# technosaurus/PDMP3

Hardware: AMD Instinct MI355X
Metric: MP3 frames/sec (44.1 kHz stereo 320 kbps), transforms-only hot path (higher is better)
Workload: dtype f32; 1 GPU; C2 (BASELINE configs[1]): 2048 stereo frames = 4096 granules per GPU per step, pre-Huffman-decoded spectra resident in HBM, one stream; frames_per_gpu=2048, granules_per_gpu=4096, seed=0x5eed0000c2, chunk_frames=auto

## Files before the change

pdmp3_amd/csrc/decode_core.h:

```cpp
#pragma once

#include <math.h>
#include <stdint.h>
#include <string.h>
#include "../../include/pdmp3_hip.h"

namespace pdmp3 {
struct ConstBank;
}

#if defined(__HIPCC__)
#define PD_FN __device__ __forceinline__
#define PD_SLOW_FN __device__ __attribute__((noinline))
#define PD_MFN __device__ __forceinline__
#define PD_HD __host__ __device__ __forceinline__
#define PD_FMA(a, b, c) __builtin_fmaf((a), (b), (c))
#define PD_CLOCK() __builtin_amdgcn_s_memtime()
#define PD_UNROLL _Pragma("unroll")
#define PD_UNROLL_N(n) _Pragma(PD_STR_(unroll n))
#define PD_STR_(x) #x
#define PD_NOUNROLL _Pragma("nounroll")
#define PD_SCHED_FENCE() __builtin_amdgcn_sched_barrier(0)
#define PD_PIN(x) asm volatile("" : "+v"(x))
#define PD_ANY(c) (__builtin_amdgcn_ballot_w64(c) != 0ull)
#define PD_LANE() ((int)(threadIdx.x & 63))
#define PD_UNIFORM(x) __builtin_amdgcn_readfirstlane((int)(x))
#define PD_SHFL_XOR(v, m) __shfl_xor((v), (m))
#define PD_WAVE_SYNC()                                       \
  __builtin_amdgcn_fence(__ATOMIC_RELEASE, "wavefront");    \
  __builtin_amdgcn_wave_barrier();                          \
  __builtin_amdgcn_fence(__ATOMIC_ACQUIRE, "wavefront")
#define PD_STORE_DEVICE(p, v) __hip_atomic_store((p), (v), __ATOMIC_RELAXED, __HIP_MEMORY_SCOPE_AGENT)
#define PD_LOAD_DEVICE(p) __hip_atomic_load((p), __ATOMIC_RELAXED, __HIP_MEMORY_SCOPE_AGENT)
#define PD_VMEM_DRAIN() asm volatile("s_waitcnt vmcnt(0)" ::: "memory")
#define PD_SLEEP() __builtin_amdgcn_s_sleep(4)
#define PD_SETPRIO(x) __builtin_amdgcn_s_setprio(x)
#define PD_LDS_FLAG(p) (*(volatile __attribute__((address_space(3))) unsigned*)(p))
#define PD_BALLOT(c) ((unsigned long long)__builtin_amdgcn_ballot_w64(c))
namespace pdmp3 {
typedef const __attribute__((address_space(4))) ConstBank* BankPtr;
}
#define PD_LAUNDER(p) asm volatile("" : "+s"(p))
#define PD_UNIFORM_PTR(T, p) ((T)(((unsigned long long)(unsigned)PD_UNIFORM((int)((unsigned long long)(p) >> 32)) << 32) | (unsigned)PD_UNIFORM((int)(unsigned long long)(p))))
#define PD_UNCHECKED_INDEX(v, lo, n) (v)
#define PD_FMED3(x, lo, hi) __builtin_amdgcn_fmed3f((x), (lo), (hi))
namespace pdmp3 {
typedef float f32x2 __attribute__((ext_vector_type(2)));
typedef unsigned short u16x2 __attribute__((ext_vector_type(2)));
typedef float f32x4 __attribute__((ext_vector_type(4)));
__device__ __forceinline__ f32x2 fma2(f32x2 a, f32x2 b, f32x2 c) { return __builtin_elementwise_fma(a, b, c); }
__device__ __forceinline__ f32x4 mfma16(float a, float b, f32x4 c) { return __builtin_amdgcn_mfma_f32_16x16x4f32(a, b, c, 0, 0, 0); }
__device__ __forceinline__ void permlane32_swap(int& a, int& b) {
  const auto r = __builtin_amdgcn_permlane32_swap((unsigned)a, (unsigned)b, false, false);
  a = (int)r[0];
  b = (int)r[1];
}
__device__ __forceinline__ void mul9_rtz_32767(const float* x, float* p) {
#define PD_M(n, m) "v_mul_f32 %" #n ", 0x46fffe00, %" #m "\n\t"
  asm volatile(
      "s_setreg_imm32_b32 hwreg(HW_REG_MODE, 0, 2), 3\n\t"
      "s_nop 1\n\t"
      PD_M(0, 9) PD_M(1, 10) PD_M(2, 11) PD_M(3, 12) PD_M(4, 13) PD_M(5, 14) PD_M(6, 15) PD_M(7, 16) PD_M(8, 17)
      "s_setreg_imm32_b32 hwreg(HW_REG_MODE, 0, 2), 0\n\t"
      "s_nop 1"
      : "=&v"(p[0]), "=&v"(p[1]), "=&v"(p[2]), "=&v"(p[3]), "=&v"(p[4]), "=&v"(p[5]), "=&v"(p[6]), "=&v"(p[7]), "=&v"(p[8])
      : "v"(x[0]), "v"(x[1]), "v"(x[2]), "v"(x[3]), "v"(x[4]), "v"(x[5]), "v"(x[6]), "v"(x[7]), "v"(x[8]));
#undef PD_M
}
__device__ __forceinline__ void mul18_rtz_32767(const float* x, float* p) {
  mul9_rtz_32767(x, p);
  mul9_rtz_32767(x + 9, p + 9);
}
}
#else
namespace pdmp3 {
// ... 5 lines not shown
bool any(bool c);
unsigned long long ballot(bool c);
void mfma16(float a, float b, float* cd);
void permlane32_swap(int* a, int* b);
}
}
#define PD_FN static inline
#define PD_SLOW_FN static
#define PD_MFN inline
#define PD_HD static inline
#define PD_FMA(a, b, c) __builtin_fmaf((a), (b), (c))
#define PD_CLOCK() 0ull
#define PD_UNROLL
#define PD_UNROLL_N(n)
#define PD_NOUNROLL
#define PD_SCHED_FENCE() ((void)0)
#define PD_PIN(x) ((void)0)
#define PD_ANY(c) (::pdmp3::emu::any(c))
#define PD_LANE() (::pdmp3::emu::lane())
#define PD_UNIFORM(x) ((int)(x))
#define PD_SHFL_XOR(v, m) (::pdmp3::emu::shfl_xor((v), (m)))
#define PD_WAVE_SYNC() ::pdmp3::emu::wave_sync()
#define PD_STORE_DEVICE(p, v) (*(p) = (v))
#define PD_LOAD_DEVICE(p) (*(p))
#define PD_VMEM_DRAIN() ::pdmp3::emu::wave_sync()
#define PD_SLEEP() ::pdmp3::emu::wave_yield()
#define PD_SETPRIO(x) ((void)0)
#define PD_LDS_FLAG(p) (*(volatile unsigned*)(p))
#define PD_BALLOT(c) (::pdmp3::emu::ballot(c))
namespace pdmp3 {
typedef const ConstBank* BankPtr;
}
#define PD_LAUNDER(p) ((void)0)
#define PD_UNIFORM_PTR(T, p) (p)
#define PD_UNCHECKED_INDEX(v, lo, n) ((unsigned)((v) - (lo)) < (unsigned)(n) ? (v) : 0)
namespace pdmp3 {
typedef float f32x2 __attribute__((vector_size(8)));
typedef unsigned short u16x2 __attribute__((vector_size(4)));
typedef float f32x4 __attribute__((vector_size(16)));
static inline f32x2 fma2(f32x2 a, f32x2 b, f32x2 c) { return (f32x2){__builtin_fmaf(a[0], b[0], c[0]), __builtin_fmaf(a[1], b[1], c[1])}; }
static inline f32x4 mfma16(float a, float b, f32x4 c) {
  float cd[4] = {c[0], c[1], c[2], c[3]};
  emu::mfma16(a, b, cd);
  return (f32x4){cd[0], cd[1], cd[2], cd[3]};
}
static inline void permlane32_swap(int& a, int& b) { emu::permlane32_swap(&a, &b); }
static inline float pd_fmed3_host(float x, float lo, float hi) {
  if (x != x) return lo < hi ? lo : hi;
  return x < lo ? lo : (x > hi ? hi : x);
}
static inline void mul18_rtz_32767(const float* x, float* p) {
  for (int t = 0; t < 18; t++) {
    const double d = (double)x[t] * 32767.0;
    float f = (float)d;
    if (f == f && !__builtin_isinf(f) && __builtin_fabs((double)f) > __builtin_fabs(d)) f = __builtin_nextafterf(f, 0.0f);
    else if (__builtin_isinf(f) && !__builtin_isinf(x[t])) f = __builtin_copysignf(0x1.fffffep+127f, f);
    p[t] = f;
  }
}
}
#define PD_FMED3(x, lo, hi) (::pdmp3::pd_fmed3_host((x), (lo), (hi)))
#endif

#ifndef PD_EXP_SKIP
#define PD_EXP_SKIP 0
#endif
// ... 174 lines not shown
  for (int m = 0; m < kOvlRegs; m++) R.ovl[m] = 0.0f;
  for (int s = 0; s < kHistSlots; s++) { R.he[s] = 0.0f; R.ho[s] = 0.0f; }
}

template <bool TAPS = true>
PD_FN void lane_init(int lane, WaveData& L, LaneRegs& R, BankPtr cb, const GlobalTables& T) {
  const int i = lane & 31;
  (void)cb;
  R.idx_e = (i < 16) ? 16 + i : ((i == 16) ? 0 : 48 - i);
  R.idx_o = (i <= 16) ? 16 - i : i - 16;
  if (TAPS) {
    for (int k = 0; k < 8; k++) {
      R.we[k] = T.taps[k * 64 + lane];
      R.wo[k] = T.taps[(8 + k) * 64 + lane];
    }
  }
  state_zero(lane, R);
  if (lane < 4) L.peek[lane] = 1.0f;
  for (int k = 0; k < 10; k++) R.bi[k] = T.frag_long[k * 64 + lane];
  for (int k = 0; k < 8; k++) R.bm[k] = T.frag_mat[k * 64 + lane];
}

PD_HD int fast_line(int lane, int i) { return i < 4 ? 2 * lane + 128 * i : 512 + lane; }
PD_FN unsigned band_addr_of(const GlobalTables& T, int sfreq, int line) {
  return (unsigned)((T.linetab[(size_t)sfreq * 3 * 576 + line] >> 10) << 2);
}

PD_FN void tab_load_image(int tid, int nthr, TabLds& S, const GlobalTables& T, int sfreq) {
  const Chunk16* src = reinterpret_cast<const Chunk16*>(reinterpret_cast<const char*>(T.tab_image) + (size_t)sfreq * sizeof(TabLds));
  Chunk16* dst = reinterpret_cast<Chunk16*>(&S);
  for (int k = tid; k < (int)(sizeof(TabLds) / 16); k += nthr) dst[k] = src[k];
}
PD_FN void load_linetab(int lane, TabLds& S, const GlobalTables& T, int sfreq) { tab_load_image(lane, 64, S, T, sfreq); }

constexpr int kStateFloats = 64 * (kOvlRegs + 2 * kHistSlots);

PD_FN void state_load(int lane, LaneRegs& R, const float* st) {
  for (int m = 0; m < kOvlRegs; m++) R.ovl[m] = st[m * 64 + lane];
  for (int s = 0; s < kHistSlots; s++) {
    R.he[s] = st[(kOvlRegs + s) * 64 + lane];
    R.ho[s] = st[(kOvlRegs + kHistSlots + s) * 64 + lane];
  }
}

PD_FN void state_load_ch1(int lane, LaneRegs& R, const float* st) {
  for (int m = 8; m < 16; m++) R.ovl[m] = st[m * 64 + lane];
  if (lane >= 32) {
    R.ovl[16] = st[16 * 64 + lane];
    R.ovl[17] = st[17 * 64 + lane];
    for (int s = 0; s < kHistSlots; s++) {
      R.he[s] = st[(kOvlRegs + s) * 64 + lane];
      R.ho[s] = st[(kOvlRegs + kHistSlots + s) * 64 + lane];
    }
  }
}

PD_FN void state_store(int lane, const LaneRegs& R, float* st) {
  for (int m = 0; m < kOvlRegs; m++) st[m * 64 + lane] = R.ovl[m];
  for (int s = 0; s < kHistSlots; s++) {
    st[(kOvlRegs + s) * 64 + lane] = R.he[s];
    st[(kOvlRegs + kHistSlots + s) * 64 + lane] = R.ho[s];
  }
}

PD_FN void ph_prefetch(int lane, LaneRegs& R, const int16_t* spectra_g, const pdmp3_gc_side* side_g) {
  const Chunk16* src = reinterpret_cast<const Chunk16*>(spectra_g);
  R.pf0 = src[lane];
  R.pf1 = src[lane + 64];
  if (lane < 16) {
    R.pf2 = src[lane + 128];
    R.pf3 = reinterpret_cast<const Chunk16*>(side_g)[lane];
  }
}

PD_FN void ph_commit(int lane, WaveData& L, const LaneRegs& R) {
  Chunk16* dst = reinterpret_cast<Chunk16*>(&L.spec[0][0]);
  dst[lane] = R.pf0;
  dst[lane + 64] = R.pf1;
  if (lane < 16) {
    dst[lane + 128] = R.pf2;
    reinterpret_cast<Chunk16*>(&L.side[0][0])[lane] = R.pf3;
  }
}

PD_HD float pow2_quarter(int k) {
  const int j = k & 3;
  const float base = (j == 0) ? 1.0f : (j == 1) ? 0x1.306fe0p+0f : (j == 2) ? 0x1.6a09e6p+0f : 0x1.ae89fap+0f;
  return ldexpf(base, k >> 2);
}
PD_HD float pow2_neg_half(uint32_t n) {
  const float v = ldexpf((n & 1) ? 0x1.6a09e6p-1f : 1.0f, -(int)((n < 300u ? n : 300u) >> 1));
  return n >= 300u ? 0.0f : v;
}

PD_FN void ph_scales(int lane, WaveData& L) {
  const bool is_long = lane < 22;
  const int ll = is_long ? lane : 21;
  const int q = is_long ? 0 : (lane < 61 ? lane - 22 : 38);
  const int sfb = q / 3, win = q - 3 * sfb;
  const int pre = (int)((0x2fe95400000ull >> (2 * ll)) & 3);
  const float pk = L.peek[win];
  float res[2];
  PD_UNROLL for (int ch = 0; ch < 2; ch++) {
    const uint8_t* s = L.side[ch];
    const int gg = s[2], flags = s[3];
// ... 724 lines not shown
  const int lane = PD_LANE();
  const unsigned long long t_wave_start = PROF ? PD_CLOCK() : 0ull;
  const int f0 = chunk * a.chunk_frames;
  int f1 = state_only ? f0 : f0 + a.chunk_frames;
  if (f1 > a.n_frames) f1 = a.n_frames;
  const int g_begin = 2 * f0;
  int g_end = 2 * f1;
  if (a.n_gran > 0 && g_end > a.n_gran) g_end = a.n_gran;
  int g_start = 0;
  int g_peek = -1;
  if (g_begin > 0) {
    const uint8_t fl = reinterpret_cast<const uint8_t*>(a.side + (size_t)(g_begin - 1) * 2 + 1)[3];
    const bool shrt = (fl & PDMP3_GC_WIN_SWITCH) && ((fl & PDMP3_GC_BLOCK_TYPE_MASK) >> PDMP3_GC_BLOCK_TYPE_SHIFT) == 2;
    g_start = g_begin - (shrt ? kHaloGranulesH5 : kHaloGranules);
    if (shrt && g_start > 0) g_peek = g_start;
    if (g_start < 0) g_start = 0;
  }
  const bool last = (f1 == a.n_frames) && !state_only;
  int pre_end = 0, npre = 0;
  int g_keep = -1;
  bool ch1_from_state = false;
  if (g_start > 0) {
    const uint8_t fb = reinterpret_cast<const uint8_t*>(a.side + (size_t)(f0 - 1) * 4)[7];
    const bool prev_mono = ((fb & PDMP3_FR_MODE_MASK) >> PDMP3_FR_MODE_SHIFT) == 3 && !(fb & PDMP3_FR_RESET);
    if (prev_mono && ((last && a.state_out) || state_only || last_stereo_or_reset(a.side, f0, f1) >= 0)) {
      const int fs = last_stereo_or_reset(a.side, 0, f0 - 1);
      if (fs < 0) ch1_from_state = true;
      else {
        const uint8_t sb = reinterpret_cast<const uint8_t*>(a.side + (size_t)fs * 4)[7];
        if (((sb & PDMP3_FR_MODE_MASK) >> PDMP3_FR_MODE_SHIFT) != 3) {
          pre_end = 2 * fs + 2;
          npre = (fs > 0 && !(sb & PDMP3_FR_RESET)) ? 3 : 2;
          if (npre == 3 && pre_end - 3 > 0) g_peek = pre_end - 3;
          if (pre_end >= g_start) { g_start = pre_end - npre; g_keep = pre_end - 1; npre = 0; pre_end = 0; }
        }
      }
    }
  }
  const int g_first = npre ? pre_end - npre : g_start;
  const bool from_stream_start = (g_first == 0);
  int cur_sfreq = reinterpret_cast<const uint8_t*>(a.side + (size_t)g_first * 2)[7] & PDMP3_FR_SFREQ_MASK;
  if (cur_sfreq > 2) cur_sfreq = 2;
  if (RARE) {
    int v = reinterpret_cast<const uint8_t*>(a.side + (size_t)g_first * 2)[offsetof(pdmp3_gc_side, lsf)] & PDMP3_LSF_VERSION_MASK;
    cur_sfreq += 3 * (v > 2 ? 2 : v);
  }

  PD_PHASE(
    ph_prefetch(lane, R, a.spectra + (size_t)g_first * 1152, a.side + (size_t)g_first * 2);
    if (OWN_TABS) load_linetab(lane, S, T, cur_sfreq);
    lane_init(lane, L, R, cb, T);
    if (a.state_in) {
      if (from_stream_start) state_load(lane, R, a.state_in);
      else if (ch1_from_state) state_load_ch1(lane, R, a.state_in);
    }
  )
  PD_PHASE(ph_commit(lane, L, R))
  PD_PHASE(ph_scales(lane, L))
  unsigned long long acc[kProfSlots] = {0, 0, 0, 0, 0, 0, 0, 0, 0, 0, 0, 0};
  unsigned long long tprev = PD_CLOCK();
  acc[11] = tprev;
#define PD_TICK(k) if (PROF) { const unsigned long long tn_ = PD_CLOCK(); acc[k] += tn_ - tprev; tprev = tn_; }
  for (int k = -npre; g_start + k < g_end; ++k) {
    const int g = k < 0 ? pre_end + k : g_start + k;
    const int g_next = k + 1 < 0 ? pre_end + k + 1 : g_start + k + 1;
    const int f = g >> 1, gr = g & 1;
    const bool emit = (k >= 0) && (g >= g_begin);
// ... 73 lines not shown
    return;
  }
  if (!DUMP && !PROF && gp) {
    const uint8_t fbl = reinterpret_cast<const uint8_t*>(a.side + (size_t)(f1 - 1) * 4)[7];
    if (((fbl & PDMP3_FR_MODE_MASK) >> PDMP3_FR_MODE_SHIFT) != 3 && !frame_is_rare(a.side + (size_t)(f1 - 1) * 4)) {
      PD_PHASE(gran_publish_regs(lane, R, a, 2 * f1 - 1, *gp))
    }
  }
}

constexpr int kGranFloats = 64 * (kOvlRegs + kHistSlots);
struct GranMb {
  unsigned free, tails_full, rows_full;
  unsigned peek_full;
  float peek_tail[3];
  unsigned pad;
};
struct GranPos {
  WaveData* wl;
  GranMb* mb;
  int w;
  int wpw;
  unsigned* tabs_ready;
  int ring;
  int g_base, g_end;
};
PD_FN int gran_next_place(const GranPos& gp) { return (gp.ring && gp.w + 1 == gp.wpw) ? 0 : gp.w + 1; }
PD_FN unsigned gran_tag(const GranPos& gp, int g) { return gp.ring ? (unsigned)(g - gp.g_base + 1) : 1u; }
static_assert(sizeof(WaveData::xr) >= kOvlRegs * 64 * sizeof(float), "tails mailbox");
static_assert(offsetof(WaveData, scale) + sizeof(WaveData::scale) - offsetof(WaveData, spec) >= kHistSlots * 64 * sizeof(float) &&
              offsetof(WaveData, xr) >= offsetof(WaveData, scale) + sizeof(WaveData::scale), "rows mailbox");
PD_FN float* gran_tails_box(WaveData& L) { return &L.xr[0][0]; }
PD_FN float* gran_rows_box(WaveData& L) { return reinterpret_cast<float*>(&L.spec[0][0]); }
PD_FN void gran_lds_flag(int lane, unsigned* p) { if (lane == 0) PD_LDS_FLAG(p) = 1u; }
PD_FN void gran_tabs_wait(const GranPos& gp) {
  while ((int)PD_UNIFORM(PD_LDS_FLAG(gp.tabs_ready)) < gp.wpw) PD_SLEEP();
  asm volatile("" ::: "memory");
}
PD_FN void gran_lds_wait(unsigned* p) {
  while (PD_UNIFORM(PD_LDS_FLAG(p)) == 0) PD_SLEEP();
  asm volatile("" ::: "memory");
}
PD_FN void gran_lds_flag_tag(int lane, unsigned* p, unsigned tag) { if (lane == 0) PD_LDS_FLAG(p) = tag; }
PD_FN void gran_lds_wait_tag(unsigned* p, unsigned tag) {
  while ((unsigned)PD_UNIFORM(PD_LDS_FLAG(p)) != tag) PD_SLEEP();
  asm volatile("" ::: "memory");
}
PD_FN void gran_far_signal(int lane, const DecodeArgs& a, int g, int k) {
  PD_VMEM_DRAIN();
  if (lane == 0) PD_STORE_DEVICE(a.chain_flag + 2 * (size_t)g + k, a.chain_epoch);
}
PD_FN void gran_send_tails(int lane, const float* y2, const DecodeArgs& a, int g, const GranPos& gp) {
  if (gp.w == gp.wpw - 1) {
    float* st = a.chain_state + (size_t)g * kGranFloats;
    for (int m = 0; m < kOvlRegs; m++) PD_STORE_DEVICE(&st[m * 64 + lane], y2[m]);
    gran_far_signal(lane, a, g, 0);
  } else {
    GranMb& mb = gp.mb[gp.w + 1];
    gran_lds_wait(&mb.free);
    float* box = gran_tails_box(gp.wl[gp.w + 1]);
    for (int m = 0; m < kOvlRegs; m++) box[m * 64 + lane] = y2[m];
    PD_WAVE_SYNC();
    gran_lds_flag(lane, &mb.tails_full);
  }
}
PD_FN void gran_send_rows(int lane, const WaveData& L, const DecodeArgs& a, int g, const GranPos& gp) {
  const int ch = lane >> 5, i = lane & 31;
  if (gp.w == gp.wpw - 1) {
    float* st = a.chain_state + (size_t)g * kGranFloats + kOvlRegs * 64;
    float v[kHistSlots];
    PD_UNROLL for (int s = 0; s < kHistSlots; s++) v[s] = L.hyb[ch][3 + s][i];
    PD_UNROLL for (int s = 0; s < kHistSlots; s++) PD_STORE_DEVICE(&st[s * 64 + lane], v[s]);
    gran_far_signal(lane, a, g, 1);
  } else {
    GranMb& mb = gp.mb[gp.w + 1];
    gran_lds_wait(&mb.free);
    float* box = gran_rows_box(gp.wl[gp.w + 1]);
    for (int s = 0; s < kHistSlots; s++) box[s * 64 + lane] = L.hyb[ch][3 + s][i];
    PD_WAVE_SYNC();
    gran_lds_flag(lane, &mb.rows_full);
  }
}
PD_FN void gran_send_tails_ring(int lane, const float* y2, int g, const GranPos& gp) {
// ... 203 lines not shown
        L.hyb[ch][t][2 * j] = me[r]; L.hyb[ch][t][2 * j + 1] = mo[r];
      }
    }
  }
}
PD_FN void ph_window_own(int lane, const WaveData& L, const TabLds& S, LaneRegs& R, float* acc) {
  const int ch = lane >> 5;
  PD_UNROLL for (int k = 0; k < 8; k++) { R.we[k] = S.taps[k][lane & 31]; R.wo[k] = S.taps[8 + k][lane & 31]; }
  float E[18], O[18];
  PD_UNROLL for (int t = 0; t < 18; t++) { E[t] = L.hyb[ch][t][R.idx_e]; O[t] = L.hyb[ch][t][R.idx_o]; }
  PD_UNROLL for (int t = 0; t < 18; t++) {
    float s = 0.0f;
    PD_UNROLL for (int k = 0; k < 8; k++) {
      if (t - 2 * k >= 0) s = PD_FMA(R.we[k], E[t - 2 * k], s);
      if (t - 2 * k - 1 >= 0) s = PD_FMA(R.wo[k], O[t - 2 * k - 1], s);
    }
    acc[t] = s;
  }
}
template <bool F32>
PD_FN void ph_window_hist(int lane, WaveData& L, const LaneRegs& R, const float* acc, int16_t* pcm_g, float* pcmf_g) {
  float sum[18];
  PD_UNROLL for (int t = 0; t < 18; t++) {
    float s = acc[t];
    PD_UNROLL for (int k = 0; k < 8; k++) {
      if (t - 2 * k < 0) s = PD_FMA(R.we[k], R.he[kHistSlots + t - 2 * k], s);
      if (t - 2 * k - 1 < 0) s = PD_FMA(R.wo[k], R.ho[kHistSlots + t - 2 * k - 1], s);
    }
    sum[t] = s;
  }
  pcm_emit<F32, true>(lane, L, 2, true, sum, pcm_g, pcmf_g);
}

template <bool F32>
PD_SLOW_FN void gran_slow_chunk(DecodeArgs a, GlobalTables T, BankPtr cb, int f, WaveData* L, TabLds* S, GranPos second, bool publish,
                                LaneRegs* state_only) {
  cb = PD_UNIFORM_PTR(BankPtr, cb);
  f = PD_UNIFORM(f);
  gran_tabs_wait(second);
  run_chunk<false, false, F32, false>(a, T, cb, f, *L, *S, publish ? &second : nullptr, state_only);
}

template <bool F32, bool RING = false>
PD_FN void run_granule(const DecodeArgs& a, const GlobalTables& T, BankPtr cb, int g, WaveData& L, TabLds& S, const GranPos& gp,
                       bool fresh, bool h5, bool next_takes, const LaneRegs& pf, LaneRegs* Rp = nullptr, bool emit = true,
                       bool zero_in = false, bool halo_in = false, int g_pf = -1) {
  LaneRegs R;
  (void)Rp;
  int lane_ = PD_LANE();
  if (RING) PD_PIN(lane_);
  const int lane = lane_;
  const int f = g >> 1, gr = g & 1;
  const bool from_caller = fresh && gr == 0 && f == 0 && a.state_in && !(reinterpret_cast<const uint8_t*>(a.side)[7] & PDMP3_FR_RESET);
  const bool from_zero = (fresh && gr == 0 && !from_caller) || (RING && zero_in);
  const bool from_chain = !from_caller && !from_zero;
  const unsigned tag = gran_tag(gp, g);
#define PD_GT(k) if (a.prof) { const unsigned long long t_ = PD_CLOCK(); if (lane == 0) a.prof[(size_t)g * kProfSlots + (k)] = t_; }
  PD_GT(1)
  R.pf0 = pf.pf0; R.pf1 = pf.pf1; R.pf2 = pf.pf2; R.pf3 = pf.pf3;
  const bool far_sender = !RING && gp.w == gp.wpw - 1 && next_takes;
  if (far_sender) PD_SETPRIO(2);
  PD_PHASE(lane_init<false>(lane, L, R, cb, T))
  if (h5 && (gr == 1 || !fresh)) {
    if (!RING) PD_SETPRIO(3);
    float pk = 0.0f;
    gran_tabs_wait(gp);
    if (gr == 0) {
      LaneRegs R1;
      R1.ovl[0] = 0.0f;
      PD_PHASE(ph_prefetch(lane, R1, a.spectra + (size_t)(g - 1) * 1152, a.side + (size_t)(g - 1) * 2))
      PD_PHASE(ph_commit(lane, L, R1))
      PD_PHASE(ph_scales(lane, L))
      PD_PHASE((ph_requant<false, 1, false, true, false, false>(lane, L, S, cb, T, nullptr, nullptr)))
      PD_PHASE(ph_antialias(lane, L, cb, true))
      PD_PHASE(ph_peek_tail(lane, L, S, R1, T))
      GranMb& mb = gp.mb[gran_next_place(gp)];
      if (lane < 3) mb.peek_tail[lane] = R1.ovl[0];
      PD_WAVE_SYNC();
      if (RING) gran_lds_flag_tag(lane, &mb.peek_full, gran_tag(gp, g + 1));
      else gran_lds_flag(lane, &mb.peek_full);
    } else {
      LaneRegs R0;
      float tail = 0.0f;
      PD_PHASE(ph_prefetch(lane, R0, a.spectra + (size_t)(g - 1) * 1152, a.side + (size_t)(g - 1) * 2))
      if (fresh && f == 0 && a.state_in && !(reinterpret_cast<const uint8_t*>(a.side)[7] & PDMP3_FR_RESET) && lane < 3) tail = a.state_in[lane];
      PD_PHASE(ph_commit(lane, L, R0))
      PD_PHASE(ph_scales(lane, L))
      PD_PHASE((ph_requant<false, 1, false, true, false, false>(lane, L, S, cb, T, nullptr, nullptr)))
      PD_PHASE(ph_antialias(lane, L, cb, true))
      const float head = ph_peek_head(lane, L, S, T);
      PD_WAVE_SYNC();
      if (!fresh) {
        if (RING) gran_lds_wait_tag(&gp.mb[gp.w].peek_full, tag);
        else gran_lds_wait(&gp.mb[gp.w].peek_full);
        tail = lane < 3 ? gp.mb[gp.w].peek_tail[lane] : 0.0f;
      }
      pk = head + tail;
    }
    PD_PHASE(ph_commit(lane, L, R))
    if (gr == 1) { PD_PHASE(if (lane < 3) L.peek[lane] = pk) }
  } else {
    PD_PHASE(ph_commit(lane, L, R))
  }
  PD_GT(2)
  gran_tabs_wait(gp);
  PD_LAUNDER(cb);
  const GranuleInfo gi = granule_info<false>(L);
  if (!(PD_EXP_SKIP & 1)) { PD_PHASE((ph_requant<false, 9, true, true, true, false>(lane, L, S, cb, T, nullptr, nullptr, &gi))) }
  PD_GT(3)
  if (!RING && !(h5 && (gr == 1 || !fresh))) {
    const int q = gp.w >> 2;
    if (q == 1) PD_SETPRIO(1); else if (q == 2) PD_SETPRIO(2); else if (q == 3) PD_SETPRIO(3); else PD_SETPRIO(0);
  }
  if (!(PD_EXP_SKIP & 2)) { PD_PHASE(ph_antialias(lane, L, cb, false, &gi)) }
  float y1[kOvlRegs], y2[kOvlRegs];
  if (PD_EXP_SKIP & 4) { PD_UNROLL for (int m = 0; m < kOvlRegs; m++) { y1[m] = L.xr[0][m * 64 + lane]; y2[m] = L.xr[1][m * 64 + lane]; } }
  else { PD_PHASE(ph_imdct(lane, L, S, R, cb, T, y1, y2, &gi)) }
  PD_GT(4)
  if (RING) gran_lds_flag_tag(lane, &gp.mb[gp.w].free, tag);
// ... 47 lines not shown
    if (from_chain) gran_lds_wait_tag(&gp.mb[gp.w].rows_full, tag);
    PD_GT(11)
    return;
  }
  float acc[18];
  if (PD_EXP_SKIP & 16) { PD_UNROLL for (int t = 0; t < 18; t++) acc[t] = L.hyb[0][t][lane & 31]; } else { PD_PHASE(ph_window_own(lane, L, S, R, acc)) }
  PD_GT(9)
  if (have_halo) { PD_UNROLL for (int s = 0; s < kHistSlots; s++) { R.he[s] = H.he[s]; R.ho[s] = H.ho[s]; } }
  else if (from_caller) {
    PD_UNROLL for (int s = 0; s < kHistSlots; s++) {
      R.he[s] = a.state_in[(kOvlRegs + s) * 64 + lane];
      R.ho[s] = a.state_in[(kOvlRegs + kHistSlots + s) * 64 + lane];
    }
  } else if (from_zero) { PD_UNROLL for (int s = 0; s < kHistSlots; s++) { R.he[s] = 0.0f; R.ho[s] = 0.0f; } }
  else if (RING || gp.w > 0) {
    if (RING) gran_lds_wait_tag(&gp.mb[gp.w].rows_full, tag);
    else gran_lds_wait(&gp.mb[gp.w].rows_full);
    const float* rows = gran_rows_box(L) + (lane >> 5) * 32;
    PD_UNROLL for (int s = 0; s < kHistSlots; s++) { R.he[s] = rows[s * 64 + R.idx_e]; R.ho[s] = rows[s * 64 + R.idx_o]; }
  } else {
    gran_far_wait(a, g, 1, false);
    const float* rows = a.chain_state + (size_t)(g - 1) * kGranFloats + kOvlRegs * 64 + (lane >> 5) * 32;
    PD_UNROLL for (int s = 0; s < kHistSlots; s++) { R.he[s] = PD_LOAD_DEVICE(&rows[s * 64 + R.idx_e]); R.ho[s] = PD_LOAD_DEVICE(&rows[s * 64 + R.idx_o]); }
  }
  (void)from_chain;
  PD_GT(10)
  if (PD_EXP_SKIP & 32) { a.pcm[(size_t)f * 2304 + gr * 1152 + lane] = (int16_t)(acc[0] + acc[17] + R.he[0] + R.ho[14]); } else { PD_PHASE(ph_window_hist<F32>(lane, L, R, acc, a.pcm + (size_t)f * 2304 + gr * 1152, F32 ? a.pcm_f32 + (size_t)f * 2304 + gr * 1152 : nullptr)) }
  PD_GT(11)
#undef PD_GT
}

template <bool F32, bool RING = false>
PD_FN void run_granule_wave(const DecodeArgs& a, const GlobalTables& T, BankPtr cb, int g, WaveData& L, TabLds& S, const GranPos& gp,
                            const LaneRegs& pf, LaneRegs* Rp = nullptr, int g_emit = 0, bool halo_by_wave = false, int g_pf = -1) {
  const int f = g >> 1, gr = g & 1;
  const uint8_t fb = reinterpret_cast<const uint8_t*>(a.side + (size_t)f * 4)[7];
  const uint8_t pb = reinterpret_cast<const uint8_t*>(a.side + (size_t)(f > 0 ? f - 1 : 0) * 4)[7];
  const uint8_t nb = reinterpret_cast<const uint8_t*>(a.side + (size_t)(f + 1 < a.n_frames ? f + 1 : f) * 4)[7];
  const uint8_t fl = reinterpret_cast<const uint8_t*>(a.side + (size_t)(2 * f + 1) * 2 + 1)[3];
  const bool rare = frame_is_rare(a.side + (size_t)f * 4);
  const bool prev_rare = frame_is_rare(a.side + (size_t)(f > 0 ? f - 1 : 0) * 4);
  const bool next_rare = frame_is_rare(a.side + (size_t)(f + 1 < a.n_frames ? f + 1 : f) * 4);
  const bool stereo = ((fb & PDMP3_FR_MODE_MASK) >> PDMP3_FR_MODE_SHIFT) != 3 && !rare;
  const bool fresh = f == 0 || (fb & PDMP3_FR_RESET);
  const bool prev_stereo = ((pb & PDMP3_FR_MODE_MASK) >> PDMP3_FR_MODE_SHIFT) != 3 && !prev_rare;
  const bool chained = stereo && (fresh || prev_stereo);
  const bool h5 = (fl & PDMP3_GC_WIN_SWITCH) && ((fl & PDMP3_GC_BLOCK_TYPE_MASK) >> PDMP3_GC_BLOCK_TYPE_SHIFT) == 2;
  bool next_takes = false;
  if (chained) {
    next_takes = gr == 0 || (f + 1 < a.n_frames && ((nb & PDMP3_FR_MODE_MASK) >> PDMP3_FR_MODE_SHIFT) != 3 && !(nb & PDMP3_FR_RESET) && !next_rare);
    if (RING) {
      if (g + 1 >= gp.g_end) next_takes = false;
      const bool halo_frame = g < g_emit;
      run_granule<F32, true>(a, T, cb, g, L, S, gp, fresh, h5, next_takes, pf, Rp, !halo_frame, halo_frame && gr == 0 && !fresh,
                             halo_by_wave && g == g_emit && !fresh, g_pf);
    } else run_granule<F32, false>(a, T, cb, g, L, S, gp, fresh, h5, next_takes, pf);
    return;
  }
  if (gr == 0) {
    GranPos second = gp;
    second.w = gp.w + 1;
    if (RING) {
      gran_slow_chunk<F32>(a, T, cb, f, &L, &S, second, true, nullptr);
    } else gran_slow_chunk<F32>(a, T, cb, f, &L, &S, second, true, nullptr);
  }
}

template <bool F32>
PD_FN void run_granule_ring(const DecodeArgs& a, const GlobalTables& T, BankPtr cb, WaveData& L, TabLds& S, GranPos gp, int f0, int f1) {
  const int lane = PD_LANE();
  int g_emit = 2 * f0;
  bool halo_by_wave = false;
  gp.ring = 1;
  gp.g_base = g_emit;
  gp.g_end = 2 * f1;
  if (f0 > 0) {
    const uint8_t b0 = reinterpret_cast<const uint8_t*>(a.side + (size_t)f0 * 4)[7];
    const uint8_t b1 = reinterpret_cast<const uint8_t*>(a.side + (size_t)(f0 - 1) * 4)[7];
    const uint8_t b2 = reinterpret_cast<const uint8_t*>(a.side + (size_t)(f0 > 1 ? f0 - 2 : 0) * 4)[7];
    const bool st0 = ((b0 & PDMP3_FR_MODE_MASK) >> PDMP3_FR_MODE_SHIFT) != 3 && !frame_is_rare(a.side + (size_t)f0 * 4);
    const bool st1 = ((b1 & PDMP3_FR_MODE_MASK) >> PDMP3_FR_MODE_SHIFT) != 3 && !frame_is_rare(a.side + (size_t)(f0 - 1) * 4);
    const bool st2 = ((b2 & PDMP3_FR_MODE_MASK) >> PDMP3_FR_MODE_SHIFT) != 3 && !frame_is_rare(a.side + (size_t)(f0 > 1 ? f0 - 2 : 0) * 4);
    const bool needs_state = st0 && !(b0 & PDMP3_FR_RESET) && st1;
    if (needs_state) {
      const bool prev_goes_granule_way = (b1 & PDMP3_FR_RESET) || f0 == 1 || st2;
      if (prev_goes_granule_way) gp.g_base = g_emit - 2;
      else halo_by_wave = true;
    }
  }
  GlobalTables Tl = T;
  for (int g = gp.g_base + gp.w; g < gp.g_end; g += gp.wpw) {
    PD_LAUNDER(Tl.taps); PD_LAUNDER(Tl.frag_long); PD_LAUNDER(Tl.frag_mat);
    if (a.prof) { const unsigned long long t_ = PD_CLOCK(); if (lane == 0) a.prof[(size_t)g * kProfSlots] = t_; }
    LaneRegs pf;
    ph_prefetch(lane, pf, a.spectra + (size_t)g * 1152, a.side + (size_t)g * 2);
    run_granule_wave<F32, true>(a, Tl, cb, g, L, S, gp, pf, nullptr, g_emit, halo_by_wave, -1);
    PD_WAVE_SYNC();
  }
}

}
```

pdmp3_amd/csrc/engine.hip:

```cpp
#include <hip/hip_runtime.h>

#include <stddef.h>
#include <stdio.h>
#include <stdlib.h>
#include <string.h>

#include "decode_core.h"
#include "engine_internal.h"
#include "gen_core.h"
#include "host_tables.h"
#include "unpack_core.h"
#include <new>

using namespace pdmp3;

#ifndef PDMP3_WAVES_PER_EU
#define PDMP3_WAVES_PER_EU 2
#endif

__constant__ ConstBank c_bank;

__device__ __forceinline__ int xcd_contiguous(int b, int n) {
  const int q = n >> 3, r = n & 7, x = b & 7;
  return (x < r ? x * (q + 1) : r * (q + 1) + (x - r) * q) + (b >> 3);
// ... 8 lines not shown
  if (chunk >= n_chunks) return;
  if (DUMP) { run_chunk<DUMP, false, F32, true, true>(a, T, (BankPtr)&c_bank, chunk, L[w], L[w].tab); return; }
  if (rare_flag && chunk_is_rare(a, chunk)) {
    if ((threadIdx.x & 63) == 0) __hip_atomic_store(rare_flag, rare_epoch, __ATOMIC_RELAXED, __HIP_MEMORY_SCOPE_AGENT);
    return;
  }
  run_chunk<DUMP, false, F32, true, false>(a, T, (BankPtr)&c_bank, chunk, L[w], L[w].tab);
}

template <bool F32>
__global__ __launch_bounds__(64, PDMP3_WAVES_PER_EU) void k_decode_rare(DecodeArgs a, GlobalTables T, int n_chunks, int always, const unsigned* rare_flag, unsigned rare_epoch) {
  __shared__ WaveLds L[1];
  const int chunk = (int)blockIdx.x;
  if (chunk >= n_chunks) return;
  if (!always) {
    if (__hip_atomic_load(rare_flag, __ATOMIC_RELAXED, __HIP_MEMORY_SCOPE_AGENT) != rare_epoch) return;
    if (!chunk_is_rare(a, chunk)) return;
  }
  run_chunk<false, false, F32, true, true>(a, T, (BankPtr)&c_bank, chunk, L[0], L[0].tab);
}

template <bool F32, int W>
__global__ __launch_bounds__(64 * W) __attribute__((amdgpu_waves_per_eu(W / 4, W / 4))) void k_decode_g(DecodeArgs a, GlobalTables T) {
  __shared__ WaveData L[W];
  __shared__ TabLds S;
  __shared__ GranMb mb[W];
  __shared__ unsigned tabs_ready;
  static_assert(sizeof(WaveData) * W + sizeof(TabLds) + sizeof(GranMb) * W + 16 <= 160 * 1024, "one workgroup of 16 waves per CU");
  const int tid = (int)threadIdx.x;
  const unsigned long long t_entry = a.prof ? PD_CLOCK() : 0ull;
  const int w = tid >> 6;
  const int g = (int)blockIdx.x * W + w;
  const bool valid = g < 2 * a.n_frames;
  LaneRegs pf;
  if (valid) ph_prefetch(tid & 63, pf, a.spectra + (size_t)g * 1152, a.side + (size_t)g * 2);
  if (tid < W * (int)(sizeof(GranMb) / 4)) reinterpret_cast<unsigned*>(mb)[tid] = 0u;
  if (tid == 0) tabs_ready = 0u;
  __syncthreads();
  tab_load_image(tid, 64 * W, S, T, a.sf_hint);
  __builtin_amdgcn_fence(__ATOMIC_RELEASE, "wavefront");
  __builtin_amdgcn_wave_barrier();
  if ((tid & 63) == 0) atomicAdd(&tabs_ready, 1u);
  if (!valid) return;
  if (a.prof && (tid & 63) == 0) a.prof[(size_t)g * kProfSlots] = t_entry;
  const GranPos gp{L, mb, w, W, &tabs_ready};
  run_granule_wave<F32>(a, T, (BankPtr)&c_bank, g, L[w], S, gp, pf);
}

#if defined(PDMP3_WITH_RING_KERNEL)
template <bool F32>
__global__ __launch_bounds__(64 * 16) __attribute__((amdgpu_waves_per_eu(4, 4))) void k_decode_p(DecodeArgs a, GlobalTables T, int frames_per_wg) {
  constexpr int W = 16;
  __shared__ WaveData L[W];
  __shared__ TabLds S;
  __shared__ GranMb mb[W];
  __shared__ unsigned tabs_ready;
  const int tid = (int)threadIdx.x;
  const int w = tid >> 6;
  if (tid < W * (int)(sizeof(GranMb) / 4)) reinterpret_cast<unsigned*>(mb)[tid] = 0u;
  if (tid == 0) tabs_ready = 0u;
  __syncthreads();
  tab_load_image(tid, 64 * W, S, T, a.sf_hint);
  __builtin_amdgcn_fence(__ATOMIC_RELEASE, "wavefront");
  __builtin_amdgcn_wave_barrier();
  if ((tid & 63) == 0) atomicAdd(&tabs_ready, 1u);
  const int f0 = (int)blockIdx.x * frames_per_wg;
  int f1 = f0 + frames_per_wg;
  if (f1 > a.n_frames) f1 = a.n_frames;
  const GranPos gp{L, mb, w, W, &tabs_ready, 1, 2 * f0, 2 * f1};
  run_granule_ring<F32>(a, T, (BankPtr)&c_bank, L[w], S, gp, f0, f1);
}
#endif

__global__ __launch_bounds__(64, PDMP3_WAVES_PER_EU) void k_decode_prof(DecodeArgs a, GlobalTables T) {
  __shared__ WaveLds L[1];
  const int w = threadIdx.x >> 6;
  run_chunk<false, true, false, true, false>(a, T, (BankPtr)&c_bank, (int)blockIdx.x, L[w], L[w].tab);
}

// ... 592 lines not shown
```

Baseline: 111.7 million frames/s.

## Hoist table image, route dwords and neighbour spectra loads ahead of barriers

The table image is now loaded into registers before the workgroup barrier and stored to LDS afterwards, so its global latency overlaps with the spectrum prefetch and mailbox init. Per-granule routing bytes (frame flags, rare checks, neighbours) are read once as uniform scalar dwords through a constant-address-space pointer instead of scattered byte loads. The previous granule's spectra prefetch for h5 is issued before lane_init. All lanes now prefetch, with invalid waves clamped to the last granule. Register pressure rises from holding the table chunks and the extra prefetch set, and the change also tweaks g_peek handling.

```diff
diff --git a/pdmp3_amd/csrc/decode_core.h b/pdmp3_amd/csrc/decode_core.h
--- a/pdmp3_amd/csrc/decode_core.h
+++ b/pdmp3_amd/csrc/decode_core.h
@@ -41,6 +41,10 @@
 typedef const __attribute__((address_space(4))) ConstBank* BankPtr;
 }
 #define PD_LAUNDER(p) asm volatile("" : "+s"(p))
+namespace pdmp3 {
+typedef const __attribute__((address_space(4))) uint32_t* ConstU32Ptr;
+}
+#define PD_CONST_U32(p) ((::pdmp3::ConstU32Ptr)(unsigned long long)(p))
 #define PD_UNIFORM_PTR(T, p) ((T)(((unsigned long long)(unsigned)PD_UNIFORM((int)((unsigned long long)(p) >> 32)) << 32) | (unsigned)PD_UNIFORM((int)(unsigned long long)(p))))
 #define PD_UNCHECKED_INDEX(v, lo, n) (v)
 #define PD_FMED3(x, lo, hi) __builtin_amdgcn_fmed3f((x), (lo), (hi))
@@ -112,6 +116,7 @@
 typedef const ConstBank* BankPtr;
 }
 #define PD_LAUNDER(p) ((void)0)
+#define PD_CONST_U32(p) (reinterpret_cast<const uint32_t*>(p))
 #define PD_UNIFORM_PTR(T, p) (p)
 #define PD_UNCHECKED_INDEX(v, lo, n) ((unsigned)((v) - (lo)) < (unsigned)(n) ? (v) : 0)
 namespace pdmp3 {
@@ -352,6 +357,22 @@
   for (int k = tid; k < (int)(sizeof(TabLds) / 16); k += nthr) dst[k] = src[k];
 }
 PD_FN void load_linetab(int lane, TabLds& S, const GlobalTables& T, int sfreq) { tab_load_image(lane, 64, S, T, sfreq); }
+template <int NTHR>
+struct TabPart {
+  Chunk16 v[((int)(sizeof(TabLds) / 16) + NTHR - 1) / NTHR];
+};
+template <int NTHR>
+PD_FN void tab_image_issue(int tid, TabPart<NTHR>& P, const GlobalTables& T, int sfreq) {
+  const Chunk16* src = reinterpret_cast<const Chunk16*>(reinterpret_cast<const char*>(T.tab_image) + (size_t)sfreq * sizeof(TabLds));
+  constexpr int n = (int)(sizeof(P.v) / sizeof(P.v[0]));
+  PD_UNROLL for (int i = 0; i < n; i++) if (tid + i * NTHR < (int)(sizeof(TabLds) / 16)) P.v[i] = src[tid + i * NTHR];
+}
+template <int NTHR>
+PD_FN void tab_image_store(int tid, TabLds& S, const TabPart<NTHR>& P) {
+  Chunk16* dst = reinterpret_cast<Chunk16*>(&S);
+  constexpr int n = (int)(sizeof(P.v) / sizeof(P.v[0]));
+  PD_UNROLL for (int i = 0; i < n; i++) if (tid + i * NTHR < (int)(sizeof(TabLds) / 16)) dst[tid + i * NTHR] = P.v[i];
+}
 
 constexpr int kStateFloats = 64 * (kOvlRegs + 2 * kHistSlots);
 
@@ -391,6 +412,14 @@
     R.pf2 = src[lane + 128];
     R.pf3 = reinterpret_cast<const Chunk16*>(side_g)[lane];
   }
+}
+
+PD_FN void ph_prefetch_all_lanes(int lane, LaneRegs& R, const int16_t* spectra_g, const pdmp3_gc_side* side_g) {
+  const Chunk16* src = reinterpret_cast<const Chunk16*>(spectra_g);
+  R.pf0 = src[lane];
+  R.pf1 = src[lane + 64];
+  R.pf2 = src[(lane & 15) + 128];
+  R.pf3 = reinterpret_cast<const Chunk16*>(side_g)[lane & 15];
 }
 
 PD_FN void ph_commit(int lane, WaveData& L, const LaneRegs& R) {
@@ -1181,7 +1210,7 @@
           pre_end = 2 * fs + 2;
           npre = (fs > 0 && !(sb & PDMP3_FR_RESET)) ? 3 : 2;
           if (npre == 3 && pre_end - 3 > 0) g_peek = pre_end - 3;
-          if (pre_end >= g_start) { g_start = pre_end - npre; g_keep = pre_end - 1; npre = 0; pre_end = 0; }
+          if (pre_end >= g_start) { if (npre == 2) g_peek = -1; g_start = pre_end - npre; g_keep = pre_end - 1; npre = 0; pre_end = 0; }
         }
       }
     }
@@ -1321,7 +1350,8 @@
               offsetof(WaveData, xr) >= offsetof(WaveData, scale) + sizeof(WaveData::scale), "rows mailbox");
 PD_FN float* gran_tails_box(WaveData& L) { return &L.xr[0][0]; }
 PD_FN float* gran_rows_box(WaveData& L) { return reinterpret_cast<float*>(&L.spec[0][0]); }
-PD_FN void gran_lds_flag(int lane, unsigned* p) { if (lane == 0) PD_LDS_FLAG(p) = 1u; }
+PD_FN bool gran_lane0(int lane) { PD_PIN(lane); return lane == 0; }
+PD_FN void gran_lds_flag(int lane, unsigned* p) { if (gran_lane0(lane)) PD_LDS_FLAG(p) = 1u; }
 PD_FN void gran_tabs_wait(const GranPos& gp) {
   while ((int)PD_UNIFORM(PD_LDS_FLAG(gp.tabs_ready)) < gp.wpw) PD_SLEEP();
   asm volatile("" ::: "memory");
@@ -1330,14 +1360,14 @@
   while (PD_UNIFORM(PD_LDS_FLAG(p)) == 0) PD_SLEEP();
   asm volatile("" ::: "memory");
 }
-PD_FN void gran_lds_flag_tag(int lane, unsigned* p, unsigned tag) { if (lane == 0) PD_LDS_FLAG(p) = tag; }
+PD_FN void gran_lds_flag_tag(int lane, unsigned* p, unsigned tag) { if (gran_lane0(lane)) PD_LDS_FLAG(p) = tag; }
 PD_FN void gran_lds_wait_tag(unsigned* p, unsigned tag) {
   while ((unsigned)PD_UNIFORM(PD_LDS_FLAG(p)) != tag) PD_SLEEP();
   asm volatile("" ::: "memory");
 }
 PD_FN void gran_far_signal(int lane, const DecodeArgs& a, int g, int k) {
   PD_VMEM_DRAIN();
-  if (lane == 0) PD_STORE_DEVICE(a.chain_flag + 2 * (size_t)g + k, a.chain_epoch);
+  if (gran_lane0(lane)) PD_STORE_DEVICE(a.chain_flag + 2 * (size_t)g + k, a.chain_epoch);
 }
 PD_FN void gran_send_tails(int lane, const float* y2, const DecodeArgs& a, int g, const GranPos& gp) {
   if (gp.w == gp.wpw - 1) {
@@ -1607,6 +1637,39 @@
   pcm_emit<F32, true>(lane, L, 2, true, sum, pcm_g, pcmf_g);
 }
 
+struct GranRoute {
+  uint32_t fb, pb, nb;
+  uint32_t fx, px, nx;
+  uint32_t h;
+};
+static_assert(offsetof(pdmp3_gc_side, frame) == 7 && offsetof(pdmp3_gc_side, lsf) == 70 && offsetof(pdmp3_gc_side, flags) == 3 &&
+              sizeof(pdmp3_gc_side) == 128, "GranRoute's dwords");
+PD_FN GranRoute gran_route_load(const DecodeArgs& a, int g) {
+  const int f = g >> 1;
+  const size_t r = (size_t)f * 128;
+  const size_t rp = (size_t)(f > 0 ? f - 1 : 0) * 128;
+  const size_t rn = (size_t)(f + 1 < a.n_frames ? f + 1 : f) * 128;
+  const auto s = PD_CONST_U32(a.side);
+  GranRoute rt;
+  rt.fb = s[r + 1];
+  rt.pb = s[rp + 1];
+  rt.nb = s[rn + 1];
+  rt.fx = s[r + 17];
+  rt.px = s[rp + 17];
+  rt.nx = s[rn + 17];
+  rt.h = s[r + 3 * 32];
+  return rt;
+}
+PD_FN void gran_route_arrive(GranRoute& rt) {
+  PD_PIN(rt.fb); PD_PIN(rt.pb); PD_PIN(rt.nb); PD_PIN(rt.fx); PD_PIN(rt.px); PD_PIN(rt.nx); PD_PIN(rt.h);
+}
+PD_HD unsigned route_frame_byte(uint32_t d1) { return d1 >> 24; }
+PD_HD bool route_is_rare(uint32_t d1, uint32_t d17) {
+  const unsigned fr = route_frame_byte(d1);
+  const bool is = ((fr & PDMP3_FR_MODE_MASK) >> PDMP3_FR_MODE_SHIFT) == 1 && (fr & (1u << PDMP3_FR_MODEEXT_SHIFT));
+  return is || ((d17 >> 16) & PDMP3_LSF_VERSION_MASK) != 0;
+}
+
 template <bool F32>
 PD_SLOW_FN void gran_slow_chunk(DecodeArgs a, GlobalTables T, BankPtr cb, int f, WaveData* L, TabLds* S, GranPos second, bool publish,
                                 LaneRegs* state_only) {
@@ -1618,7 +1681,7 @@
 
 template <bool F32, bool RING = false>
 PD_FN void run_granule(const DecodeArgs& a, const GlobalTables& T, BankPtr cb, int g, WaveData& L, TabLds& S, const GranPos& gp,
-                       bool fresh, bool h5, bool next_takes, const LaneRegs& pf, LaneRegs* Rp = nullptr, bool emit = true,
+                       bool fresh, bool h5, bool next_takes, unsigned fr, const LaneRegs& pf, LaneRegs* Rp = nullptr, bool emit = true,
                        bool zero_in = false, bool halo_in = false, int g_pf = -1) {
   LaneRegs R;
   (void)Rp;
@@ -1626,15 +1689,17 @@
   if (RING) PD_PIN(lane_);
   const int lane = lane_;
   const int f = g >> 1, gr = g & 1;
-  const bool from_caller = fresh && gr == 0 && f == 0 && a.state_in && !(reinterpret_cast<const uint8_t*>(a.side)[7] & PDMP3_FR_RESET);
+  const bool from_caller = fresh && gr == 0 && f == 0 && a.state_in && !(fr & PDMP3_FR_RESET);
   const bool from_zero = (fresh && gr == 0 && !from_caller) || (RING && zero_in);
   const bool from_chain = !from_caller && !from_zero;
   const unsigned tag = gran_tag(gp, g);
-#define PD_GT(k) if (a.prof) { const unsigned long long t_ = PD_CLOCK(); if (lane == 0) a.prof[(size_t)g * kProfSlots + (k)] = t_; }
+#define PD_GT(k) if (a.prof) { const unsigned long long t_ = PD_CLOCK(); if (gran_lane0(lane)) a.prof[(size_t)g * kProfSlots + (k)] = t_; }
   PD_GT(1)
   R.pf0 = pf.pf0; R.pf1 = pf.pf1; R.pf2 = pf.pf2; R.pf3 = pf.pf3;
   const bool far_sender = !RING && gp.w == gp.wpw - 1 && next_takes;
   if (far_sender) PD_SETPRIO(2);
+  LaneRegs Rq;
+  if (h5 && (gr == 1 || !fresh)) ph_prefetch(lane, Rq, a.spectra + (size_t)(g - 1) * 1152, a.side + (size_t)(g - 1) * 2);
   PD_PHASE(lane_init<false>(lane, L, R, cb, T))
   if (h5 && (gr == 1 || !fresh)) {
     if (!RING) PD_SETPRIO(3);
@@ -1643,8 +1708,7 @@
     if (gr == 0) {
       LaneRegs R1;
       R1.ovl[0] = 0.0f;
-      PD_PHASE(ph_prefetch(lane, R1, a.spectra + (size_t)(g - 1) * 1152, a.side + (size_t)(g - 1) * 2))
-      PD_PHASE(ph_commit(lane, L, R1))
+      PD_PHASE(ph_commit(lane, L, Rq))
       PD_PHASE(ph_scales(lane, L))
       PD_PHASE((ph_requant<false, 1, false, true, false, false>(lane, L, S, cb, T, nullptr, nullptr)))
       PD_PHASE(ph_antialias(lane, L, cb, true))
@@ -1655,11 +1719,9 @@
       if (RING) gran_lds_flag_tag(lane, &mb.peek_full, gran_tag(gp, g + 1));
       else gran_lds_flag(lane, &mb.peek_full);
     } else {
-      LaneRegs R0;
       float tail = 0.0f;
-      PD_PHASE(ph_prefetch(lane, R0, a.spectra + (size_t)(g - 1) * 1152, a.side + (size_t)(g - 1) * 2))
-      if (fresh && f == 0 && a.state_in && !(reinterpret_cast<const uint8_t*>(a.side)[7] & PDMP3_FR_RESET) && lane < 3) tail = a.state_in[lane];
-      PD_PHASE(ph_commit(lane, L, R0))
+      if (fresh && f == 0 && a.state_in && !(fr & PDMP3_FR_RESET) && lane < 3) tail = a.state_in[lane];
+      PD_PHASE(ph_commit(lane, L, Rq))
       PD_PHASE(ph_scales(lane, L))
       PD_PHASE((ph_requant<false, 1, false, true, false, false>(lane, L, S, cb, T, nullptr, nullptr)))
       PD_PHASE(ph_antialias(lane, L, cb, true))
@@ -1773,15 +1835,14 @@
 
 template <bool F32, bool RING = false>
 PD_FN void run_granule_wave(const DecodeArgs& a, const GlobalTables& T, BankPtr cb, int g, WaveData& L, TabLds& S, const GranPos& gp,
-                            const LaneRegs& pf, LaneRegs* Rp = nullptr, int g_emit = 0, bool halo_by_wave = false, int g_pf = -1) {
+                            const LaneRegs& pf, const GranRoute& rt, LaneRegs* Rp = nullptr, int g_emit = 0, bool halo_by_wave = false,
+                            int g_pf = -1) {
   const int f = g >> 1, gr = g & 1;
-  const uint8_t fb = reinterpret_cast<const uint8_t*>(a.side + (size_t)f * 4)[7];
-  const uint8_t pb = reinterpret_cast<const uint8_t*>(a.side + (size_t)(f > 0 ? f - 1 : 0) * 4)[7];
-  const uint8_t nb = reinterpret_cast<const uint8_t*>(a.side + (size_t)(f + 1 < a.n_frames ? f + 1 : f) * 4)[7];
-  const uint8_t fl = reinterpret_cast<const uint8_t*>(a.side + (size_t)(2 * f + 1) * 2 + 1)[3];
-  const bool rare = frame_is_rare(a.side + (size_t)f * 4);
-  const bool prev_rare = frame_is_rare(a.side + (size_t)(f > 0 ? f - 1 : 0) * 4);
-  const bool next_rare = frame_is_rare(a.side + (size_t)(f + 1 < a.n_frames ? f + 1 : f) * 4);
+  const unsigned fb = route_frame_byte(rt.fb), pb = route_frame_byte(rt.pb), nb = route_frame_byte(rt.nb);
+  const unsigned fl = rt.h >> 24;
+  const bool rare = route_is_rare(rt.fb, rt.fx);
+  const bool prev_rare = route_is_rare(rt.pb, rt.px);
+  const bool next_rare = route_is_rare(rt.nb, rt.nx);
   const bool stereo = ((fb & PDMP3_FR_MODE_MASK) >> PDMP3_FR_MODE_SHIFT) != 3 && !rare;
   const bool fresh = f == 0 || (fb & PDMP3_FR_RESET);
   const bool prev_stereo = ((pb & PDMP3_FR_MODE_MASK) >> PDMP3_FR_MODE_SHIFT) != 3 && !prev_rare;
@@ -1793,9 +1854,9 @@
     if (RING) {
       if (g + 1 >= gp.g_end) next_takes = false;
       const bool halo_frame = g < g_emit;
-      run_granule<F32, true>(a, T, cb, g, L, S, gp, fresh, h5, next_takes, pf, Rp, !halo_frame, halo_frame && gr == 0 && !fresh,
+      run_granule<F32, true>(a, T, cb, g, L, S, gp, fresh, h5, next_takes, fb, pf, Rp, !halo_frame, halo_frame && gr == 0 && !fresh,
                              halo_by_wave && g == g_emit && !fresh, g_pf);
-    } else run_granule<F32, false>(a, T, cb, g, L, S, gp, fresh, h5, next_takes, pf);
+    } else run_granule<F32, false>(a, T, cb, g, L, S, gp, fresh, h5, next_takes, fb, pf);
     return;
   }
   if (gr == 0) {
@@ -1805,6 +1866,13 @@
       gran_slow_chunk<F32>(a, T, cb, f, &L, &S, second, true, nullptr);
     } else gran_slow_chunk<F32>(a, T, cb, f, &L, &S, second, true, nullptr);
   }
+}
+template <bool F32, bool RING = false>
+PD_FN void run_granule_wave(const DecodeArgs& a, const GlobalTables& T, BankPtr cb, int g, WaveData& L, TabLds& S, const GranPos& gp,
+                            const LaneRegs& pf, LaneRegs* Rp = nullptr, int g_emit = 0, bool halo_by_wave = false, int g_pf = -1) {
+  GranRoute rt = gran_route_load(a, PD_UNIFORM(g));
+  gran_route_arrive(rt);
+  run_granule_wave<F32, RING>(a, T, cb, g, L, S, gp, pf, rt, Rp, g_emit, halo_by_wave, g_pf);
 }
 
 template <bool F32>
@@ -1833,9 +1901,11 @@
   for (int g = gp.g_base + gp.w; g < gp.g_end; g += gp.wpw) {
     PD_LAUNDER(Tl.taps); PD_LAUNDER(Tl.frag_long); PD_LAUNDER(Tl.frag_mat);
     if (a.prof) { const unsigned long long t_ = PD_CLOCK(); if (lane == 0) a.prof[(size_t)g * kProfSlots] = t_; }
+    GranRoute rt = gran_route_load(a, PD_UNIFORM(g));
     LaneRegs pf;
     ph_prefetch(lane, pf, a.spectra + (size_t)g * 1152, a.side + (size_t)g * 2);
-    run_granule_wave<F32, true>(a, Tl, cb, g, L, S, gp, pf, nullptr, g_emit, halo_by_wave, -1);
+    gran_route_arrive(rt);
+    run_granule_wave<F32, true>(a, Tl, cb, g, L, S, gp, pf, rt, nullptr, g_emit, halo_by_wave, -1);
     PD_WAVE_SYNC();
   }
 }
diff --git a/pdmp3_amd/csrc/engine.hip b/pdmp3_amd/csrc/engine.hip
--- a/pdmp3_amd/csrc/engine.hip
+++ b/pdmp3_amd/csrc/engine.hip
@@ -64,19 +64,25 @@
   const int w = tid >> 6;
   const int g = (int)blockIdx.x * W + w;
   const bool valid = g < 2 * a.n_frames;
+  TabPart<64 * W> tp;
+  tab_image_issue<64 * W>(tid, tp, T, a.sf_hint);
+  GranRoute rt;
+  if (valid) rt = gran_route_load(a, (int)blockIdx.x * W + PD_UNIFORM(w));
   LaneRegs pf;
-  if (valid) ph_prefetch(tid & 63, pf, a.spectra + (size_t)g * 1152, a.side + (size_t)g * 2);
+  const int g_in = valid ? g : 2 * a.n_frames - 1;
+  ph_prefetch_all_lanes(tid & 63, pf, a.spectra + (size_t)g_in * 1152, a.side + (size_t)g_in * 2);
   if (tid < W * (int)(sizeof(GranMb) / 4)) reinterpret_cast<unsigned*>(mb)[tid] = 0u;
   if (tid == 0) tabs_ready = 0u;
   __syncthreads();
-  tab_load_image(tid, 64 * W, S, T, a.sf_hint);
+  tab_image_store<64 * W>(tid, S, tp);
   __builtin_amdgcn_fence(__ATOMIC_RELEASE, "wavefront");
   __builtin_amdgcn_wave_barrier();
   if ((tid & 63) == 0) atomicAdd(&tabs_ready, 1u);
   if (!valid) return;
   if (a.prof && (tid & 63) == 0) a.prof[(size_t)g * kProfSlots] = t_entry;
   const GranPos gp{L, mb, w, W, &tabs_ready};
-  run_granule_wave<F32>(a, T, (BankPtr)&c_bank, g, L[w], S, gp, pf);
+  gran_route_arrive(rt);
+  run_granule_wave<F32>(a, T, (BankPtr)&c_bank, g, L[w], S, gp, pf, rt);
 }
 
 #if defined(PDMP3_WITH_RING_KERNEL)
```

Result: no change. 112.5 million frames/s (median of 6 runs) (+0.8%).
